# joybio/multiPrime

Measured on AMD Instinct MI355X. Metric: candidate x sequence coverage evals/s, higher is better.
Workload: dtype u32; 1 GPU; synthetic MSA 1048576 x 1000, k=18, v=1, 8 candidates/window, 950 windows, strict -c 2,3,-1 per GPU x 1 GPU(s) = BASELINE configs[3] itself (SURVEY 8d input 4; synthetic 1M x 1 kb; shape 1x1: row shards x window groups); rows_per_gpu=1048576, rows_total=1048576, cols=1000, k=18, variation=1, candidates_per_window=8, windows=950, parallelism=one GPU holds every row

## Files before the change

multiprime_amd/csrc/chainbody.hpp:

```cpp
#pragma once

#include "common.hpp"
#include "bitslice.hpp"

namespace mp {

struct EvalChainArgs {
    const unsigned long long *cols;
    const unsigned long long *excl;
    int nw, p0, k, v;
    const ChainItem *items;
    const uint32_t *events;
    const int32_t *cand_out;
    uint32_t sF, sR;
    unsigned long long *out;
    BlockMap map;
    PatchArgs patch;
    const ChainItem *neg_items;
    int n_neg;
    unsigned long long *clear;
    uint32_t n_clear;
};

__device__ __forceinline__ void clear_counters(unsigned long long *__restrict__ p, uint32_t n, unsigned bid, unsigned n_blocks) {
    if (!p) return;
    for (uint32_t i = bid * kBlock + threadIdx.x; i < n; i += n_blocks * kBlock) p[i] = 0ull;
}

template <int LV, int GW, int D, int NB>
__device__ __forceinline__ void chain_first_pass(uint32_t rem, const uint32_t *Pw, size_t nw32, unsigned long long sy_lo,
                                                 unsigned long long sy_hi, uint32_t sF, uint32_t sR, uint32_t (&t1)[GW],
                                                 uint32_t (&t2)[GW], uint32_t (&t3)[GW], uint32_t (&t4)[GW], uint32_t (&sf)[GW],
                                                 uint32_t (&sr)[GW]) {
#pragma unroll 1
    while (rem) {
        int js[D]; bool has[D];
        uint32_t ld[D][NB][GW], sys[D];
#pragma unroll
        for (int u = 0; u < D; u++) {
            has[u] = rem != 0u;
            js[u] = has[u] ? __builtin_ctz(rem) : js[0];
            rem &= rem - 1u;
            const int j = js[u];
            const uint32_t sy = (uint32_t)((j < 16 ? sy_lo : sy_hi) >> (4 * (j & 15))) & 15u;
            sys[u] = sy;
            const uint32_t *P = Pw + (size_t)j * 4 * nw32;
            if (NB == 4) {
#pragma unroll
                for (int b = 0; b < 4; b++)
#pragma unroll
                    for (int i = 0; i < GW; i++) ld[u][b][i] = P[b * nw32 + i];
            } else {
                const uint32_t second = sy & (sy - 1u);
                const size_t b0 = (size_t)__builtin_ctz(sy | 16u), b1 = (size_t)__builtin_ctz(second | 16u);
#pragma unroll
                for (int i = 0; i < GW; i++) {
                    ld[u][0][i] = P[b0 * nw32 + i];
                    if (NB == 2) ld[u][1][i] = P[b1 * nw32 + i];
                }
            }
        }
#pragma unroll
        for (int u = 0; u < D; u++) {
            if (!has[u]) break;
            const int j = js[u];
            uint32_t m[GW];
            if (NB == 4) {
                const uint32_t sy = sys[u];
                const uint32_t kA = (sy & 1u) ? 0xFFFFFFFFu : 0u, kC = (sy & 2u) ? 0xFFFFFFFFu : 0u;
                const uint32_t kG = (sy & 4u) ? 0xFFFFFFFFu : 0u, kT = (sy & 8u) ? 0xFFFFFFFFu : 0u;
#pragma unroll
                for (int i = 0; i < GW; i++) {
                    m[i] = ld[u][0][i] & kA;
                    m[i] = __builtin_amdgcn_bitop3_b32(ld[u][1][i], kC, m[i], kLutAndOr);
                    m[i] = __builtin_amdgcn_bitop3_b32(ld[u][2][i], kG, m[i], kLutAndOr);
                    m[i] = __builtin_amdgcn_bitop3_b32(ld[u][3][i], kT, m[i], kLutAndOr);
                }
            } else {
#pragma unroll
                for (int i = 0; i < GW; i++) m[i] = NB == 2 ? (ld[u][0][i] | ld[u][1][i]) : ld[u][0][i];
            }
#pragma unroll
            for (int i = 0; i < GW; i++) count_unmatched<LV>(t1[i], t2[i], t3[i], t4[i], m[i]);
            if (((sF | sR) >> j) & 1u) {
                const uint32_t fF = ((sF >> j) & 1u) ? 0xFFFFFFFFu : 0u, fR = ((sR >> j) & 1u) ? 0xFFFFFFFFu : 0u;
#pragma unroll
                for (int i = 0; i < GW; i++) {
                    sf[i] = __builtin_amdgcn_bitop3_b32(sf[i], m[i], fF, kLutOrNotAnd);
                    sr[i] = __builtin_amdgcn_bitop3_b32(sr[i], m[i], fR, kLutOrNotAnd);
                }
            }
        }
    }
}

template <int LV, int GW, int D>
__device__ __forceinline__ void eval_chain_block(const EvalChainArgs &A, uint32_t (&s_part)[kBlock / 64][12], const unsigned bid) {
    static_assert(GW <= 8, "plane rows are padded to multiples of 8 words");
    constexpr int CC = 8;
    const int patch_blocks = A.patch.n_blocks + A.patch.neg_blocks;
    const bool on_patch = (int)bid < patch_blocks;
    const bool negative = on_patch && (int)bid >= A.patch.n_blocks;
    int slice, item, word0;
    if (on_patch) {
        const int pb = (int)bid - (negative ? A.patch.n_blocks : 0);
        const int unit = __builtin_amdgcn_readfirstlane(pb * (kBlock / 64) + (int)(threadIdx.x >> 6));
        item = unit / A.patch.per_item;
        slice = unit % A.patch.per_item;
        if (item >= (negative ? A.n_neg : A.map.n_items)) return;
        word0 = (slice * 64 + (int)(threadIdx.x & 63)) * GW;
    } else {
        if (!map_block(A.map, bid - (unsigned)patch_blocks, slice, item)) return;
        word0 = (slice * kBlock + threadIdx.x) * GW;
    }
    const ChainItem it = negative ? A.neg_items[item] : A.items[item];
    const WordTile T = !on_patch ? column_tile(A.cols, A.excl, A.nw, A.p0, it.win, word0)
                                 : (negative ? plain_tile(A.patch, it.win, word0) : patch_tile(A.patch, it.win, word0));
    if (on_patch && slice * 64 * GW >= (int)T.stride) return;
    const size_t nw32 = T.stride;
    const bool live = T.live;
    static_assert(32 * GW < 1024, "three counts per register need 10 bits each");
    uint32_t acc[CC];
#pragma unroll
    for (int c = 0; c < CC; c++) acc[c] = 0;
    if (live) {
        uint32_t t1[GW], t2[GW], t3[GW], t4[GW], sf[GW], sr[GW];
#pragma unroll
        for (int i = 0; i < GW; i++) t1[i] = t2[i] = t3[i] = t4[i] = sf[i] = sr[i] = 0;
        const uint32_t *Pw = T.planes;
        const unsigned long long sy_lo = it.sym[0] | ((unsigned long long)it.sym[1] << 32);
        const unsigned long long sy_hi = it.sym[2] | ((unsigned long long)it.sym[3] << 32);
        chain_first_pass<LV, GW, D, 1>(it.pos1, Pw, nw32, sy_lo, sy_hi, A.sF, A.sR, t1, t2, t3, t4, sf, sr);
        chain_first_pass<LV, GW, (D + 1) / 2, 2>(it.pos2, Pw, nw32, sy_lo, sy_hi, A.sF, A.sR, t1, t2, t3, t4, sf, sr);
        chain_first_pass<LV, GW, (D + 3) / 4, 4>(it.pos4, Pw, nw32, sy_lo, sy_hi, A.sF, A.sR, t1, t2, t3, t4, sf, sr);
        uint32_t valid[GW];
        {
#pragma unroll
            for (int i = 0; i < GW; i++) valid[i] = T.mask[i] ^ T.mask_flip;
        }
        const uint32_t *ev = A.events + it.ev0;
        int e = 0;
        uint32_t evw = it.n_ev ? ev[0] : (1u << 8);
        uint32_t cur[GW];
        {
            const uint32_t *P = Pw + ((size_t)(evw & 255u) * 4 + (size_t)__builtin_ctz(((evw >> 8) & 15u) | 16u)) * nw32;
#pragma unroll
            for (int i = 0; i < GW; i++) cur[i] = P[i];
        }
#pragma unroll
        for (int s = 0; s < CC; s++) {
            if (s >= it.n_steps) break;
            if (s > 0) {
#pragma unroll 1
                while (e < it.n_ev && (int)(evw >> 16) == s) {
                    e++;
                    const uint32_t evn = e < it.n_ev ? ev[e] : evw;
                    uint32_t nxt[GW];
                    {
                        const uint32_t *P = Pw + ((size_t)(evn & 255u) * 4 + (size_t)__builtin_ctz(((evn >> 8) & 15u) | 16u)) * nw32;
#pragma unroll
                        for (int i = 0; i < GW; i++) nxt[i] = P[i];
                    }
                    const uint32_t j = evw & 255u;
#pragma unroll
                    for (int i = 0; i < GW; i++) count_plane<LV>(t1[i], t2[i], t3[i], t4[i], cur[i]);
                    if (((A.sF | A.sR) >> j) & 1u) {
                        const uint32_t fF = ((A.sF >> j) & 1u) ? 0xFFFFFFFFu : 0u, fR = ((A.sR >> j) & 1u) ? 0xFFFFFFFFu : 0u;
#pragma unroll
                        for (int i = 0; i < GW; i++) {
                            sf[i] = __builtin_amdgcn_bitop3_b32(sf[i], cur[i], fF, kLutOrAnd);
                            sr[i] = __builtin_amdgcn_bitop3_b32(sr[i], cur[i], fR, kLutOrAnd);
                        }
                    }
#pragma unroll
                    for (int i = 0; i < GW; i++) cur[i] = nxt[i];
                    evw = evn;
                }
            }
            uint32_t nP = 0, nF = 0, nR = 0;
#pragma unroll
            for (int i = 0; i < GW; i++) {
                const uint32_t far = LV == 1 ? t1[i] : (LV == 2 ? t2[i] : (LV == 3 ? t3[i] : t4[i]));
                nP += __popc(valid[i] & ~t1[i]);
                nF += __popc(__builtin_amdgcn_bitop3_b32(valid[i], far, sf[i], kLutAndNotNot));
                nR += __popc(__builtin_amdgcn_bitop3_b32(valid[i], far, sr[i], kLutAndNotNot));
            }
            acc[s] = nP | (nF << 10) | (nR << 20);
        }
    }
    uint32_t accP[CC], accF[CC], accR[CC];
#pragma unroll
    for (int c = 0; c < CC; c++) { accP[c] = acc[c] & 1023u; accF[c] = (acc[c] >> 10) & 1023u; accR[c] = acc[c] >> 20; }
    if (on_patch) wave_commit<GW>(accP, accF, accR, s_part[threadIdx.x >> 6], A.cand_out + it.cand0, A.out, negative);
    else block_commit<GW>(accP, accF, accR, s_part, A.cand_out + it.cand0, A.out);
}

constexpr int kPatchEvents = 16;
template <int LV>
__device__ __forceinline__ void eval_patch_wave(const EvalChainArgs &A, uint32_t *row, uint32_t *stash, const unsigned unit, const bool negative) {
    constexpr int CC = 8, GW = 1;
    const int lane = (int)(threadIdx.x & 63);
    const int item = __builtin_amdgcn_readfirstlane((int)(unit / (unsigned)A.patch.per_item)), slice = __builtin_amdgcn_readfirstlane((int)(unit % (unsigned)A.patch.per_item));
    if (item >= (negative ? A.n_neg : A.map.n_items)) return;
    const int word0 = slice * 64 + lane;
    const ChainItem it = negative ? A.neg_items[item] : A.items[item];
    const WordTile T = negative ? plain_tile(A.patch, it.win, word0) : patch_tile(A.patch, it.win, word0);
    if (slice * 64 >= (int)T.stride) return;
    const size_t nw32 = T.stride;
    const uint32_t *Pw = T.planes;
    const uint32_t *ev = A.events + it.ev0;
    const int n_ev = __builtin_amdgcn_readfirstlane((int)it.n_ev), n_steps = __builtin_amdgcn_readfirstlane((int)it.n_steps);
    const uint32_t evv = lane < n_ev ? ev[lane] : 0u;
    uint32_t acc[CC];
#pragma unroll
    for (int c = 0; c < CC; c++) acc[c] = 0;
    const uint32_t *Pl = T.live ? Pw : Pw - (word0 - slice * 64) ;
    uint32_t t1[GW] = {0}, t2[GW] = {0}, t3[GW] = {0}, t4[GW] = {0}, sf[GW] = {0}, sr[GW] = {0};
    const unsigned long long sy_lo = it.sym[0] | ((unsigned long long)it.sym[1] << 32);
    const unsigned long long sy_hi = it.sym[2] | ((unsigned long long)it.sym[3] << 32);
    chain_first_pass<LV, GW, 16, 1>(it.pos1, Pl, nw32, sy_lo, sy_hi, A.sF, A.sR, t1, t2, t3, t4, sf, sr);
    chain_first_pass<LV, GW, 8, 2>(it.pos2, Pl, nw32, sy_lo, sy_hi, A.sF, A.sR, t1, t2, t3, t4, sf, sr);
    chain_first_pass<LV, GW, 4, 4>(it.pos4, Pl, nw32, sy_lo, sy_hi, A.sF, A.sR, t1, t2, t3, t4, sf, sr);
    const uint32_t valid = T.live ? (T.mask[0] ^ T.mask_flip) : 0u;
    auto plane_of = [&](uint32_t evw) { return Pl + ((size_t)(evw & 255u) * 4 + (size_t)__builtin_ctz(((evw >> 8) & 15u) | 16u)) * nw32; };
    {
        uint32_t pl[kPatchEvents];
#pragma unroll
        for (int u = 0; u < kPatchEvents; u++) {
            const int e = n_ev ? (u < n_ev ? u : n_ev - 1) : 0;
            const uint32_t evw = n_ev ? (uint32_t)__builtin_amdgcn_readlane((int)evv, e) : (1u << 8);
            pl[u] = plane_of(evw)[0];
        }
#pragma unroll
        for (int u = 0; u < kPatchEvents; u++) stash[u * 64 + lane] = pl[u];
    }
    int e = 0;
#pragma unroll
    for (int s = 0; s < CC; s++) {
        if (s >= n_steps) break;
        if (s > 0) {
#pragma unroll 1
            while (e < n_ev) {
                const uint32_t evw = e < 64 ? (uint32_t)__builtin_amdgcn_readlane((int)evv, e) : ev[e];
                if ((int)(evw >> 16) != s) break;
                const uint32_t cur = e < kPatchEvents ? stash[e * 64 + lane] : plane_of(evw)[0];
                const uint32_t j = evw & 255u;
                count_plane<LV>(t1[0], t2[0], t3[0], t4[0], cur);
                if (((A.sF | A.sR) >> j) & 1u) {
                    const uint32_t fF = ((A.sF >> j) & 1u) ? 0xFFFFFFFFu : 0u, fR = ((A.sR >> j) & 1u) ? 0xFFFFFFFFu : 0u;
                    sf[0] = __builtin_amdgcn_bitop3_b32(sf[0], cur, fF, kLutOrAnd);
                    sr[0] = __builtin_amdgcn_bitop3_b32(sr[0], cur, fR, kLutOrAnd);
                }
                e++;
            }
        }
        const uint32_t far = LV == 1 ? t1[0] : (LV == 2 ? t2[0] : (LV == 3 ? t3[0] : t4[0]));
        const uint32_t nP = (uint32_t)__popc(valid & ~t1[0]);
        const uint32_t nF = (uint32_t)__popc(__builtin_amdgcn_bitop3_b32(valid, far, sf[0], kLutAndNotNot));
        const uint32_t nR = (uint32_t)__popc(__builtin_amdgcn_bitop3_b32(valid, far, sr[0], kLutAndNotNot));
        acc[s] = nP | (nF << 10) | (nR << 20);
    }
    uint32_t accP[CC], accF[CC], accR[CC];
#pragma unroll
    for (int c = 0; c < CC; c++) { accP[c] = acc[c] & 1023u; accF[c] = (acc[c] >> 10) & 1023u; accR[c] = acc[c] >> 20; }
    wave_commit<GW>(accP, accF, accR, row, A.cand_out + it.cand0, A.out, negative);
}

}
```

multiprime_amd/csrc/common.hpp:

```cpp
#pragma once

#include "../../include/mprime.h"

#include <hip/hip_runtime.h>

#include <algorithm>
#include <cstdarg>
#include <cstdio>
#include <cstdlib>
#include <cstring>
#include <numeric>
#include <utility>
#include <chrono>
#include <mutex>
#include <unordered_map>
#include <vector>

namespace mp {

constexpr int kBlock = 256;
constexpr uint32_t kEmpty = 0xFFFFFFFFu;
constexpr int kHashSlots = 4096;
constexpr int kHashLimit = 3584;
constexpr int kEvalCC = 8;
// ... 115 lines not shown
    uint32_t *pplanes = nullptr, *pvalid = nullptr;
    uint32_t *qplanes = nullptr, *qvalid = nullptr;
    bool qp_dirty = true;
    mp::PatchWin *pwin = nullptr;
    size_t pp_words = 0, pv_words = 0;
    int max_npw = 0;
    bool pp_dirty = true;
    unsigned long long *g_key = nullptr;
    uint32_t *g_cnt = nullptr, *g_min = nullptr;
    uint32_t *g_gap = nullptr;
    int32_t *g_idx = nullptr;
    int g_slots = 0;
    long long u_cap = 0, u_n = 0;
    uint32_t *u_b0 = nullptr, *u_b1 = nullptr, *u_g = nullptr;
    int32_t *u_count = nullptr, *u_first = nullptr, *labels = nullptr, *u_over = nullptr, *u_wcount = nullptr;
    int64_t *u_wbase = nullptr;
    unsigned long long *u_total = nullptr;
    std::vector<int64_t> h_wbase;
    std::vector<int32_t> h_wcount;
    double gate_threshold = 0;
    std::vector<uint8_t> h_wskip;
    uint8_t *dm_loss = nullptr;
    double *dm_dg = nullptr;
    std::vector<uint8_t> dm_loss_host;
    std::vector<double> dm_dg_host;
    unsigned long long *mask_f = nullptr, *mask_r = nullptr;
    size_t mask_words = 0;
    int n_masks = 0;
    int n_cand = 0, n_items = 0, n_padded = 0;
    mp::EvalItem *items = nullptr;
    uint4 *cand_n = nullptr;
    uint32_t *cand_symT = nullptr, *cand_diff = nullptr, *chain_events = nullptr;
    mp::ChainItem *chain_items = nullptr;
    void *x_items = nullptr;
    uint32_t *x_events = nullptr;
    int32_t *x_cand_out = nullptr;
    int x_n = 0, x_n_events = 0;
    int32_t *table_ids = nullptr;
    int n_chain = 0, n_table = 0, n_events = 0, max_steps = 0;
    std::vector<mp::ChainItem> h_chains;
    std::vector<uint32_t> h_events;
    std::vector<int32_t> h_cand_out;
    uint32_t *chain_prog = nullptr;
    size_t chain_prog_n = 0;
    mp::EvalForm form;
    mp::SlideBand *slide_bands = nullptr;
    uint32_t *slide_iters = nullptr, *slide_recs = nullptr;
    size_t slide_n_iters = 0;
    int slide_items = 0, slide_n_bands = 0, slide_max_items = 0, slide_ns = 0, slide_gw = 0;
    uint32_t slide_spos = 0, slide_fmask = 0, slide_rmask = 0, slide_fpos = 0, slide_rpos = 0;
    bool slide_fast = false;
    mp::ChainItem *chain_rest = nullptr;
    mp::ChainItem *chain_slid = nullptr;
    int n_rest = 0, rest_max_steps = 0;
    unsigned launch_seq = 0;
    int32_t *cand_out = nullptr;
    uint64_t sF = 0, sR = 0;
    unsigned long long *tmp_out = nullptr;
    int tmp_out_n = 0;
    struct PoolBlock { void *p; size_t bytes; hipEvent_t released; };
    std::vector<hipEvent_t> pool_events;
    std::unordered_map<void *, size_t> pool_live;
    std::vector<PoolBlock> pool;
    size_t pool_bytes = 0;
    long long pool_hits = 0, pool_misses = 0;
    int pool_on = -1;
    std::mutex pool_mu;
    unsigned long long *stats_buf = nullptr;
    size_t stats_buf_n = 0;
    std::vector<std::pair<hipEvent_t, hipEvent_t>> ev_busy, ev_free;
    double ev_ms = 0;
    std::vector<float> ev_samples, ev_last;
    int ev_n = 0;
    uint8_t *h_stage = nullptr;
    size_t h_stage_bytes = 0;
    bool h_stage_pinned = false;
    uint8_t *h_stats = nullptr;
    size_t h_stats_bytes = 0, stats_pending_f = 0, stats_pending_t = 0;
    bool h_stats_pinned = false;
    hipEvent_t stats_ev = nullptr;
    uint8_t *h_ring = nullptr;
    bool h_ring_pinned = false;
    hipEvent_t h_ring_ev[3] = {nullptr, nullptr, nullptr};
    uint8_t *sq_bytes = nullptr;
    int64_t *sq_roff = nullptr;
    unsigned long long *sq_code = nullptr, *sq_flag = nullptr;
    int64_t *sq_woff = nullptr;
    int32_t sq_n = 0;
    size_t sq_total = 0, sq_words = 0;
    std::vector<int64_t> sq_roff_host;
    int32_t *ot_out = nullptr;
    int64_t ot_n = 0;
    std::vector<uint8_t> ot_key;
    double ot_ms[4] = {0, 0, 0, 0};
    int64_t ot_counts[7] = {0, 0, 0, 0, 0, 0, 0};
    uint8_t *an_code = nullptr;
    uint32_t *an_kmer = nullptr;
    int32_t *an_table = nullptr;
    int32_t *an_col = nullptr, *an_colinv = nullptr;
    int32_t an_n = 0, an_L = 0, an_slots = 0;
    int32_t an_par[6] = {0, 0, 0, 0, 0, 0};
    double an_ms[5] = {0, 0, 0, 0, 0};
    int64_t an_counts[3] = {0, 0, 0};
    int32_t an_both = 0;
    uint8_t *cl_code = nullptr;
    int64_t *cl_off = nullptr;
// ... 127 lines not shown
```

multiprime_amd/csrc/evalslide.hip:

```cpp
#include "common.hpp"
#include "bitslice.hpp"
#include "slidecore.hpp"
#include "evalslide.hpp"
#include "chainbody.hpp"

using namespace mp;

namespace {

typedef unsigned int u32x4 __attribute__((ext_vector_type(4)));
typedef unsigned int u32x2 __attribute__((ext_vector_type(2)));

struct SlideKernArgs {
    SlideArgs A;
    const uint32_t *cols32;
    const uint32_t *excl32;
    int nw32;
    unsigned long long *out;
    int wc, wc_pad;
    int max_items;
    int n_slide_blocks;
    EvalChainArgs chain;
    unsigned long long *clear;
    uint32_t n_clear;
    int patch_words;
    unsigned long long *stamps;
};

template <int GW>
struct DevEnv {
    const SlideKernArgs &K;
    __amdgpu_buffer_rsrc_t rs_cols, rs_excl;
    int voff, lane;
    uint32_t row_bytes;
    bool live;
    uint32_t *ring;
    uint32_t *tab;
    uint32_t itv;
    uint32_t live_mask;

    __device__ __forceinline__ DevEnv(const SlideKernArgs &k) : K(k) {}
    __device__ __forceinline__ void progress(int quarter) const {
#ifndef SLIDE_NO_PRIO
        if (quarter <= 0) __builtin_amdgcn_s_setprio(3);
        else if (quarter == 1) __builtin_amdgcn_s_setprio(2);
        else if (quarter == 2) __builtin_amdgcn_s_setprio(1);
        else __builtin_amdgcn_s_setprio(0);
#endif
    }
    __device__ __forceinline__ void stamp(int i) const {
        if (K.stamps && threadIdx.x == 0) K.stamps[(size_t)blockIdx.x * 8 + i] = wall_clock64();
    }
    __device__ __forceinline__ SlideBand uband(int b) const {
        const SlideBand *p = K.A.bands + b;
        SlideBand r;
        r.w0 = __builtin_amdgcn_readfirstlane(p->w0); r.n_win = __builtin_amdgcn_readfirstlane(p->n_win);
        r.item0 = __builtin_amdgcn_readfirstlane(p->item0); r.n_items = __builtin_amdgcn_readfirstlane(p->n_items);
        r.iter0 = __builtin_amdgcn_readfirstlane(p->iter0); r.pad = 0;
        return r;
    }
    __device__ __forceinline__ void load_iters(int idx) { itv = K.A.iters[(size_t)idx + (size_t)lane]; }
    __device__ __forceinline__ uint32_t iter_word(int j) const { return (uint32_t)__builtin_amdgcn_readlane((int)itv, j); }
    typedef const uint32_t __attribute__((address_space(4))) * ConstWords;
    struct Rec { uint32_t w[8], sm_lo, sm_hi, flags; ConstWords p; };
    __device__ __forceinline__ Rec load_rec(int item) const {
        Rec r;
        r.p = (ConstWords)(K.A.recs + (size_t)__builtin_amdgcn_readfirstlane(item) * kSlideRec);
#pragma unroll
        for (int q = 0; q < 8; q++) r.w[q] = r.p[q];
        r.sm_lo = r.p[24]; r.sm_hi = r.p[25]; r.flags = r.p[28];
        return r;
    }
    __device__ __forceinline__ uint32_t rec_word(const Rec &r, int q) const {
        return q < 8 ? r.w[q] : (q == 24 ? r.sm_lo : (q == 25 ? r.sm_hi : (q == 28 ? r.flags : r.p[q])));
    }
    __device__ __forceinline__ uint32_t rec_word_dyn(const Rec &r, int q) const { return r.p[q]; }
    template <int AUX = 0>
    __device__ __forceinline__ void load(__amdgpu_buffer_rsrc_t rs, int soff, uint32_t (&d)[GW]) const {
        if constexpr (GW == 4) {
            const u32x4 v = __builtin_amdgcn_raw_buffer_load_b128(rs, voff, soff, AUX);
// ... 51 lines not shown
        asm volatile(
            "s_nop 1\n\t"
            "v_add_u32_dpp %0, %0, %0 row_ror:4 row_mask:0xf bank_mask:0x5\n\t"
            "v_add_u32_dpp %2, %2, %2 row_ror:4 row_mask:0xf bank_mask:0x5\n\t"
            "v_add_u32_dpp %4, %4, %4 row_ror:4 row_mask:0xf bank_mask:0x5\n\t"
            "v_add_u32_dpp %6, %6, %6 row_ror:4 row_mask:0xf bank_mask:0x5\n\t"
            "v_add_u32_dpp %8, %8, %8 row_ror:4 row_mask:0xf bank_mask:0x5\n\t"
            "v_add_u32_dpp %10, %10, %10 row_ror:4 row_mask:0xf bank_mask:0x5\n\t"
            "v_add_u32_dpp %0, %1, %1 row_ror:4 row_mask:0xf bank_mask:0xa\n\t"
            "v_add_u32_dpp %2, %3, %3 row_ror:4 row_mask:0xf bank_mask:0xa\n\t"
            "v_add_u32_dpp %4, %5, %5 row_ror:4 row_mask:0xf bank_mask:0xa\n\t"
            "v_add_u32_dpp %6, %7, %7 row_ror:4 row_mask:0xf bank_mask:0xa\n\t"
            "v_add_u32_dpp %8, %9, %9 row_ror:4 row_mask:0xf bank_mask:0xa\n\t"
            "v_add_u32_dpp %10, %11, %11 row_ror:4 row_mask:0xf bank_mask:0xa\n\t"
            "v_add_u32_dpp %0, %0, %0 row_ror:8 row_mask:0xf bank_mask:0x3\n\t"
            "v_add_u32_dpp %4, %4, %4 row_ror:8 row_mask:0xf bank_mask:0x3\n\t"
            "v_add_u32_dpp %8, %8, %8 row_ror:8 row_mask:0xf bank_mask:0x3\n\t"
            "v_add_u32_dpp %0, %2, %2 row_ror:8 row_mask:0xf bank_mask:0xc\n\t"
            "v_add_u32_dpp %4, %6, %6 row_ror:8 row_mask:0xf bank_mask:0xc\n\t"
            "v_add_u32_dpp %8, %10, %10 row_ror:8 row_mask:0xf bank_mask:0xc\n\t"
            "v_add_u32_dpp %0, %0, %0 quad_perm:[1,0,3,2] row_mask:0xf bank_mask:0xf\n\t"
            "v_add_u32_dpp %4, %4, %4 quad_perm:[1,0,3,2] row_mask:0xf bank_mask:0xf\n\t"
            "v_add_u32_dpp %8, %8, %8 quad_perm:[1,0,3,2] row_mask:0xf bank_mask:0xf\n\t"
            "v_add_u32_dpp %0, %0, %0 quad_perm:[2,3,0,1] row_mask:0xf bank_mask:0xf\n\t"
            "v_add_u32_dpp %4, %4, %4 quad_perm:[2,3,0,1] row_mask:0xf bank_mask:0xf\n\t"
            "v_add_u32_dpp %8, %8, %8 quad_perm:[2,3,0,1] row_mask:0xf bank_mask:0xf\n\t"
            "s_nop 1"
            : "+v"(x0), "+v"(x1), "+v"(x2), "+v"(x3), "+v"(x4), "+v"(x5), "+v"(x6), "+v"(x7), "+v"(x8), "+v"(x9), "+v"(x10), "+v"(x11));
        typedef unsigned int u32pair __attribute__((ext_vector_type(2)));
        const u32pair s01 = __builtin_amdgcn_permlane16_swap(x0, x4, false, false);
        const uint32_t a = s01.x + s01.y;
        const u32pair s22 = __builtin_amdgcn_permlane16_swap(x8, x8, false, false);
        const uint32_t b = s22.x + s22.y;
        const u32pair h = __builtin_amdgcn_permlane32_swap(a, b, false, false);
        const uint32_t tot = h.x + h.y;
        if (lane < 48 && (lane & 3) == 0) atomicAdd(&tab[idx * 12 + (lane >> 4) * 4 + ((lane >> 2) & 3)], tot);
    }
};

#ifndef SLIDE_MIN_WAVES
#define SLIDE_MIN_WAVES 1
#endif
template <int LV, int GW, bool FAST>
__global__ __launch_bounds__(kBlock, GW == 4 ? 1 : SLIDE_MIN_WAVES) void eval_slide_kernel(const SlideKernArgs K) {
    extern __shared__ __align__(16) uint32_t lds[];
    clear_counters(K.clear, K.n_clear, blockIdx.x, gridDim.x);
    if (K.stamps && threadIdx.x == 0) K.stamps[(size_t)blockIdx.x * 8] = wall_clock64();
    if ((int)blockIdx.x >= K.n_slide_blocks) {
        const unsigned pb = blockIdx.x - (unsigned)K.n_slide_blocks, wv = threadIdx.x >> 6;
#ifndef SLIDE_PATCH_PRIO
#define SLIDE_PATCH_PRIO 3
#endif
        __builtin_amdgcn_s_setprio(SLIDE_PATCH_PRIO);
        if (K.patch_words == 1) {
            const bool negative = (int)pb >= K.chain.patch.n_blocks;
            const unsigned unit = (pb - (negative ? (unsigned)K.chain.patch.n_blocks : 0u)) * (kBlock / 64) + wv;
            eval_patch_wave<LV>(K.chain, lds + wv * 12, lds + 64 + wv * (64 * kPatchEvents), unit, negative);
        } else {
            uint32_t(&s_part)[kBlock / 64][12] = *reinterpret_cast<uint32_t(*)[kBlock / 64][12]>(lds);
            eval_chain_block<LV, 8, 4>(K.chain, s_part, pb);
        }
        if (K.stamps && threadIdx.x == 0) K.stamps[(size_t)blockIdx.x * 8 + 7] = wall_clock64();
        return;
    }
    const int slice = (int)(blockIdx.x % (unsigned)K.wc_pad), band = (int)(blockIdx.x / (unsigned)K.wc_pad);
    if (slice >= K.wc) return;
    const int wv = (int)(threadIdx.x >> 6), lane = (int)(threadIdx.x & 63);
    const int ring_words = K.A.k * 64 * GW;
    uint32_t *tab = lds + (kBlock / 64) * ring_words;
    DevEnv<GW> env(K);
    env.lane = lane;
    env.ring = lds + wv * ring_words + lane * GW;
    env.tab = tab;
    env.itv = 0u;
    const int word0 = (slice * kBlock + (int)threadIdx.x) * GW;
    env.live = word0 < K.nw32;
    env.voff = env.live ? word0 * 4 : 0x7FFFFF00;
    env.live_mask = env.live ? 0xFFFFFFFFu : 0u;
    env.row_bytes = (uint32_t)K.nw32 * 4u;
    env.rs_cols = __builtin_amdgcn_make_buffer_rsrc(const_cast<uint32_t *>(K.cols32), 0, 0x7FFFFF00, 0x00020000);
    env.rs_excl = __builtin_amdgcn_make_buffer_rsrc(const_cast<uint32_t *>(K.excl32), 0, 0x7FFFFF00, 0x00020000);
    const SlideBand bd = env.uband(band);
    for (int i = (int)threadIdx.x; i < bd.n_items * 12; i += kBlock) tab[i] = 0u;
    __syncthreads();
    env.stamp(1);
    const bool wave_live = (slice * kBlock + wv * 64) * GW < K.nw32;
    if (wave_live) slide_band<LV, GW, true, false, FAST>(env, K.A, band);
    env.stamp(4);
    __syncthreads();
    env.stamp(5);
    int live_waves = 0;
    for (int w = 0; w < kBlock / 64; w++) live_waves += (slice * kBlock + w * 64) * GW < K.nw32 ? 1 : 0;
    const uint32_t rows = (uint32_t)live_waves * 64u * 32u * GW;
    const int n_entries = bd.n_items * 24;
    for (int i0 = (int)threadIdx.x; i0 < n_entries; i0 += 4 * kBlock) {
        int oc[4];
        uint32_t map[4];
#pragma unroll
        for (int u = 0; u < 4; u++) {
            const int i = i0 + u * kBlock, ic = i < n_entries ? i : (int)threadIdx.x;
            const uint32_t *rec = K.A.recs + (size_t)(bd.item0 + ic / 24) * kSlideRec;
            oc[u] = (int)rec[8 + (ic % 24) / 3];
            map[u] = rec[26];
        }
#pragma unroll
        for (int u = 0; u < 4; u++) {
            const int i = i0 + u * kBlock;
            if (i >= n_entries || oc[u] < 0) continue;
            const int item = i / 24, r = i % 24, t = r / 3, kind = r % 3;
            const int slot = (int)((map[u] >> (4 * t)) & 15u);
            const uint32_t *row = tab + item * 12;
            const uint32_t out1 = row[slot] & 0xFFFFu, outF = row[slot] >> 16, outR = (row[8 + (slot >> 1)] >> (16 * (slot & 1))) & 0xFFFFu;
            const uint32_t val = kind == 0 ? rows - out1 : out1 - (kind == 1 ? outF : outR);
            if (val) atomicAdd(&K.out[(size_t)oc[u] * 3 + kind], (unsigned long long)val);
        }
    }
    env.stamp(6);
}

typedef void (*SlideFn)(const SlideKernArgs);

}

namespace mp {

void free_slide(mp_ctx *c) {
    dev_free(c, &c->slide_bands, (size_t)c->slide_n_bands);
    dev_free(c, &c->slide_iters, c->slide_n_iters);
    dev_free(c, &c->slide_recs, (size_t)c->slide_items * kSlideRec);
    dev_free(c, &c->chain_rest, (size_t)c->n_rest);
    dev_free(c, &c->chain_slid, (size_t)c->slide_items);
    c->slide_items = c->slide_n_bands = c->slide_max_items = 0;
    c->slide_n_iters = 0;
    c->n_rest = c->rest_max_steps = 0;
}

int upload_eval_slide(mp_ctx *c, const std::vector<ChainItem> &chains, const std::vector<uint32_t> &events, const std::vector<int32_t> &cand_out) {
    free_slide(c);
    const char *se = getenv("MP_EVAL_SLIDE");
    if (chains.empty() || c->v > 3 || c->k <= c->v || (se ? atoi(se) != 1 : c->n_pad <= 262144)) return MP_OK;
    const int nw32 = c->n_pad / 32, n_cols = c->n_chunks * 32;
    if (((unsigned long long)n_cols * 4ull + 1ull) * (unsigned long long)nw32 * 4ull >= 0x7FFFFFFFull) return MP_OK;
    if ((unsigned long long)c->n_win * (unsigned long long)nw32 * 4ull >= 0x7FFFFFFFull) return MP_OK;
    int gw = 2;
    if (const char *e = getenv("MP_SLIDE_GW")) { const int g = atoi(e); if (g == 1 || g == 2 || g == 4) gw = g; }
    const int wc = (nw32 + kBlock * gw - 1) / (kBlock * gw), wc_pad = wc >= 8 ? (wc + 7) / 8 * 8 : wc;
    const int span = chains.back().win - chains.front().win + 1;
    std::vector<SlideChainIn> in(chains.size());
    for (size_t i = 0; i < chains.size(); i++) {
        const ChainItem &ch = chains[i];
        in[i] = SlideChainIn{ch.win, ch.cand0, ch.n_steps, ch.ev0, ch.n_ev, {ch.sym[0], ch.sym[1], ch.sym[2], ch.sym[3]}};
    }
    const size_t ring_bytes = (size_t)(kBlock / 64) * ((size_t)c->k * 64 * gw) * sizeof(uint32_t), lds_cu = 160 * 1024;
    int resident = (int)std::min<size_t>(4, std::max<size_t>(1, lds_cu / (ring_bytes + 1024)));
    if (gw == 4) resident = 1;
    SlidePlan P;
    for (;; resident--) {
        const int per_round = std::max(1, 256 * resident / std::max(1, wc_pad));
        int band = (span + per_round - 1) / per_round;
        for (int r = 2; band > 96; r++) band = (span + per_round * r - 1) / (per_round * r);
        band = std::max(8, band);
        if (const char *e = getenv("MP_SLIDE_BAND")) band = std::max(1, atoi(e));
        if (!build_slide_plan(in, events, cand_out, c->k, (uint32_t)c->sF, (uint32_t)c->sR, c->p0, n_cols, band, (uint32_t)nw32 * 4u, true, P)) return MP_OK;
        const size_t need = ring_bytes + (size_t)P.max_items_band * 12 * sizeof(uint32_t);
        if (resident <= 1 || need * (size_t)resident <= lds_cu) break;
    }
    P.iters.resize(P.iters.size() + 64, 0u);
    int rc;
    if ((rc = dev_alloc(c, &c->slide_bands, P.bands.size()))) return rc;
    c->slide_n_bands = (int)P.bands.size();
    if ((rc = dev_alloc(c, &c->slide_iters, P.iters.size()))) return rc;
    c->slide_n_iters = P.iters.size();
    c->slide_items = (int)P.item_of.size();
    if ((rc = dev_alloc(c, &c->slide_recs, P.recs.size()))) return rc;
    HIPCK(c, hipMemcpy(c->slide_bands, P.bands.data(), sizeof(SlideBand) * P.bands.size(), hipMemcpyHostToDevice));
    HIPCK(c, hipMemcpy(c->slide_iters, P.iters.data(), sizeof(uint32_t) * P.iters.size(), hipMemcpyHostToDevice));
    HIPCK(c, hipMemcpy(c->slide_recs, P.recs.data(), sizeof(uint32_t) * P.recs.size(), hipMemcpyHostToDevice));
    c->slide_max_items = P.max_items_band;
    c->slide_ns = P.ns; c->slide_spos = P.spos; c->slide_fmask = P.fmask; c->slide_rmask = P.rmask;
    c->slide_fast = slide_strict_lists(c->k, (uint32_t)c->sF, (uint32_t)c->sR, c->slide_fpos, c->slide_rpos);
    if (const char *e = getenv("MP_SLIDE_STRICT")) { if (atoi(e) == 0) c->slide_fast = false; }
    c->slide_gw = gw;
    {
        std::vector<ChainItem> slid;
        for (int32_t i : P.item_of) slid.push_back(chains[(size_t)i]);
        if ((rc = dev_alloc(c, &c->chain_slid, slid.size()))) return rc;
        HIPCK(c, hipMemcpy(c->chain_slid, slid.data(), sizeof(ChainItem) * slid.size(), hipMemcpyHostToDevice));
    }
    if (!P.rest.empty()) {
        std::vector<ChainItem> rest;
        for (int32_t i : P.rest) { rest.push_back(chains[(size_t)i]); c->rest_max_steps = std::max(c->rest_max_steps, (int)chains[(size_t)i].n_steps); }
        if ((rc = dev_alloc(c, &c->chain_rest, rest.size()))) return rc;
        c->n_rest = (int)rest.size();
        HIPCK(c, hipMemcpy(c->chain_rest, rest.data(), sizeof(ChainItem) * rest.size(), hipMemcpyHostToDevice));
    }
    return MP_OK;
}

int launch_eval_slide(mp_ctx *c, unsigned long long *device_out, const EvalChainArgs *patch, int patch_blocks, int patch_words,
                      unsigned long long *clear, uint32_t n_clear) {
#define SLIDE_ROW(LV, F) {eval_slide_kernel<LV, 1, F>, eval_slide_kernel<LV, 2, F>, eval_slide_kernel<LV, 4, F>}
    static const SlideFn fn[2][4][3] = {{SLIDE_ROW(1, false), SLIDE_ROW(2, false), SLIDE_ROW(3, false), SLIDE_ROW(4, false)},
                                        {SLIDE_ROW(1, true), SLIDE_ROW(2, true), SLIDE_ROW(3, true), SLIDE_ROW(4, true)}};
#undef SLIDE_ROW
    const int gw = c->slide_gw, gi = gw == 4 ? 2 : gw - 1;
    const int nw32 = c->n_pad / 32;
    SlideKernArgs K;
    K.A = SlideArgs{c->slide_bands, c->slide_iters, c->slide_recs, c->k, c->p0, c->slide_ns, c->slide_spos, c->slide_fmask, c->slide_rmask,
                    (uint32_t)nw32 * 4u, c->slide_fpos, c->slide_rpos, 0u, 0u};
    if (c->slide_fast) slide_strict_distinct(c->slide_fpos, c->slide_rpos, K.A.dpos, K.A.dshape);
    K.cols32 = reinterpret_cast<const uint32_t *>(c->cols);
    K.excl32 = reinterpret_cast<const uint32_t *>(c->excl);
    K.nw32 = nw32;
    K.out = device_out;
    K.wc = (nw32 + kBlock * gw - 1) / (kBlock * gw);
    K.wc_pad = K.wc >= 8 ? (K.wc + 7) / 8 * 8 : K.wc;
    K.max_items = c->slide_max_items;
    K.n_slide_blocks = c->slide_n_bands * K.wc_pad;
    if (patch) K.chain = *patch;
    else { memset(&K.chain, 0, sizeof K.chain); patch_blocks = 0; }
    K.chain.clear = nullptr; K.chain.n_clear = 0;
    K.clear = clear; K.n_clear = n_clear;
    K.patch_words = patch_words;
    K.stamps = nullptr;
    const char *stamp_file = getenv("MP_EXPERIMENT_STAMPS");
    const size_t n_stamp = ((size_t)K.n_slide_blocks + (size_t)patch_blocks) * 8;
    if (stamp_file) {
        HIPCK(c, hipMalloc(&K.stamps, n_stamp * sizeof(unsigned long long)));
        HIPCK(c, hipMemsetAsync(K.stamps, 0, n_stamp * sizeof(unsigned long long), c->stream));
    }
    size_t lds = ((size_t)(kBlock / 64) * ((size_t)c->k * 64 * gw) + (size_t)c->slide_max_items * 12) * sizeof(uint32_t);
    if (patch_blocks) lds = std::max(lds, (size_t)(64 + (kBlock / 64) * 64 * kPatchEvents) * sizeof(uint32_t));
    if (lds > 160 * 1024) return fail(c, MP_ERR_ARG, "sliding evaluation: a band needs %zu bytes of LDS", lds);
    SlideFn f = fn[c->slide_fast ? 1 : 0][c->v][gi];
    if (lds > 48 * 1024) HIPCK(c, hipFuncSetAttribute(reinterpret_cast<const void *>(f), hipFuncAttributeMaxDynamicSharedMemorySize, (int)lds));
    hipLaunchKernelGGL(f, dim3((unsigned)K.n_slide_blocks + (unsigned)patch_blocks), dim3(kBlock), lds, c->stream, K);
    HIPCK(c, hipGetLastError());
    if (stamp_file) {
        std::vector<unsigned long long> h(n_stamp + 2);
        HIPCK(c, hipStreamSynchronize(c->stream));
        HIPCK(c, hipMemcpy(h.data() + 2, K.stamps, n_stamp * sizeof(unsigned long long), hipMemcpyDeviceToHost));
        HIPCK(c, hipFree(K.stamps));
        h[0] = (unsigned long long)K.n_slide_blocks; h[1] = (unsigned long long)patch_blocks;
        if (FILE *fo = fopen(stamp_file, "wb")) { fwrite(h.data(), sizeof(unsigned long long), h.size(), fo); fclose(fo); }
    }
    return MP_OK;
}

}
```

Measured before the change: 66790 billion evals/s.

## Fuse positive and negative patch units into one signed evaluation pass

```diff
diff --git a/multiprime_amd/csrc/chainbody.hpp b/multiprime_amd/csrc/chainbody.hpp
--- a/multiprime_amd/csrc/chainbody.hpp
+++ b/multiprime_amd/csrc/chainbody.hpp
@@ -20,18 +20,24 @@
     int n_neg;
     unsigned long long *clear;
     uint32_t n_clear;
+    const uint32_t *slid_bits;
 };
+
+#ifndef PATCH_SIGNED
+#define PATCH_SIGNED 1
+#endif
 
 __device__ __forceinline__ void clear_counters(unsigned long long *__restrict__ p, uint32_t n, unsigned bid, unsigned n_blocks) {
     if (!p) return;
     for (uint32_t i = bid * kBlock + threadIdx.x; i < n; i += n_blocks * kBlock) p[i] = 0ull;
 }
 
-template <int LV, int GW, int D, int NB>
+template <int LV, int GW, int D, int NB, bool PAIR = false>
 __device__ __forceinline__ void chain_first_pass(uint32_t rem, const uint32_t *Pw, size_t nw32, unsigned long long sy_lo,
                                                  unsigned long long sy_hi, uint32_t sF, uint32_t sR, uint32_t (&t1)[GW],
                                                  uint32_t (&t2)[GW], uint32_t (&t3)[GW], uint32_t (&t4)[GW], uint32_t (&sf)[GW],
-                                                 uint32_t (&sr)[GW]) {
+                                                 uint32_t (&sr)[GW], const uint32_t *Pw2 = nullptr) {
+    static_assert(!PAIR || GW % 2 == 0, "a pair of tiles: half of the words of each");
 #pragma unroll 1
     while (rem) {
         int js[D]; bool has[D];
@@ -44,19 +50,20 @@
             const int j = js[u];
             const uint32_t sy = (uint32_t)((j < 16 ? sy_lo : sy_hi) >> (4 * (j & 15))) & 15u;
             sys[u] = sy;
-            const uint32_t *P = Pw + (size_t)j * 4 * nw32;
+            const uint32_t *P = Pw + (size_t)j * 4 * nw32, *P2 = PAIR ? Pw2 + (size_t)j * 4 * nw32 : nullptr;
+            auto word = [&](size_t b, int i) { return PAIR && i >= GW / 2 ? P2[b * nw32 + (i - GW / 2)] : P[b * nw32 + i]; };
             if (NB == 4) {
 #pragma unroll
                 for (int b = 0; b < 4; b++)
 #pragma unroll
-                    for (int i = 0; i < GW; i++) ld[u][b][i] = P[b * nw32 + i];
+                    for (int i = 0; i < GW; i++) ld[u][b][i] = word((size_t)b, i);
             } else {
                 const uint32_t second = sy & (sy - 1u);
                 const size_t b0 = (size_t)__builtin_ctz(sy | 16u), b1 = (size_t)__builtin_ctz(second | 16u);
 #pragma unroll
                 for (int i = 0; i < GW; i++) {
-                    ld[u][0][i] = P[b0 * nw32 + i];
-                    if (NB == 2) ld[u][1][i] = P[b1 * nw32 + i];
+                    ld[u][0][i] = word(b0, i);
+                    if (NB == 2) ld[u][1][i] = word(b1, i);
                 }
             }
         }
@@ -94,21 +101,59 @@
     }
 }
 
-template <int LV, int GW, int D>
-__device__ __forceinline__ void eval_chain_block(const EvalChainArgs &A, uint32_t (&s_part)[kBlock / 64][12], const unsigned bid) {
+constexpr int kPatchRowSigned = 24;
+template <int GW>
+__device__ __forceinline__ void wave_commit_signed(const uint32_t (&acc_pos)[8], const uint32_t (&acc_neg)[8], uint32_t *row, const int32_t *cand_out,
+                                                   unsigned long long *out) {
+    constexpr int CC = 8;
+    static_assert(64 * 32 * GW < 65536, "packed wave sums must fit 16 bits");
+    const int lane = threadIdx.x & 63;
+#pragma unroll
+    for (int side = 0; side < 2; side++) {
+        const uint32_t(&acc)[8] = side ? acc_neg : acc_pos;
+        uint32_t vals[3 * CC];
+#pragma unroll
+        for (int c = 0; c < CC; c++) { vals[3 * c] = acc[c] & 1023u; vals[3 * c + 1] = (acc[c] >> 10) & 1023u; vals[3 * c + 2] = acc[c] >> 20; }
+#pragma unroll
+        for (int q = 0; q < 3 * CC / 2; q++) {
+            const uint32_t tot = wave_sum_lane63(vals[2 * q] | (vals[2 * q + 1] << 16));
+            if (lane == 63) row[side * 12 + q] = tot;
+        }
+    }
+    __builtin_amdgcn_fence(__ATOMIC_RELEASE, "wavefront");
+    __builtin_amdgcn_wave_barrier();
+    __builtin_amdgcn_fence(__ATOMIC_ACQUIRE, "wavefront");
+    if (lane < 3 * CC) {
+        const int c = lane / 3, r = lane % 3;
+        auto field = [&](const uint32_t *w, int idx) { return (w[idx >> 1] >> (16 * (idx & 1))) & 0xFFFFu; };
+        const uint32_t pos = r ? field(row, lane) - field(row, 3 * c) : field(row, lane);
+        const uint32_t neg = r ? field(row + 12, lane) - field(row + 12, 3 * c) : field(row + 12, lane);
+        const int oc = cand_out[c];
+        if (oc >= 0 && pos != neg) atomicAdd(&out[(size_t)oc * 3 + r], (unsigned long long)pos - (unsigned long long)neg);
+    }
+}
+
+template <int LV, int GW, int D, bool PAIR = false>
+__device__ __forceinline__ void eval_chain_block(const EvalChainArgs &A, uint32_t (&s_part)[kBlock / 64][12], const unsigned bid, uint32_t *pair_row = nullptr) {
     static_assert(GW <= 8, "plane rows are padded to multiples of 8 words");
-    constexpr int CC = 8;
+    constexpr int CC = 8, H = PAIR ? GW / 2 : GW;
     const int patch_blocks = A.patch.n_blocks + A.patch.neg_blocks;
-    const bool on_patch = (int)bid < patch_blocks;
-    const bool negative = on_patch && (int)bid >= A.patch.n_blocks;
+    const bool on_patch = PAIR || (int)bid < patch_blocks;
+    const bool negative = !PAIR && on_patch && (int)bid >= A.patch.n_blocks;
     int slice, item, word0;
     if (on_patch) {
         const int pb = (int)bid - (negative ? A.patch.n_blocks : 0);
         const int unit = __builtin_amdgcn_readfirstlane(pb * (kBlock / 64) + (int)(threadIdx.x >> 6));
-        item = unit / A.patch.per_item;
-        slice = unit % A.patch.per_item;
-        if (item >= (negative ? A.n_neg : A.map.n_items)) return;
-        word0 = (slice * 64 + (int)(threadIdx.x & 63)) * GW;
+        if (PAIR) {
+            item = unit % A.map.n_items;
+            slice = unit / A.map.n_items;
+            if (slice >= A.patch.per_item) return;
+        } else {
+            item = unit / A.patch.per_item;
+            slice = unit % A.patch.per_item;
+            if (item >= (negative ? A.n_neg : A.map.n_items)) return;
+        }
+        word0 = (slice * 64 + (int)(threadIdx.x & 63)) * H;
     } else {
         if (!map_block(A.map, bid - (unsigned)patch_blocks, slice, item)) return;
         word0 = (slice * kBlock + threadIdx.x) * GW;
@@ -116,37 +161,51 @@
     const ChainItem it = negative ? A.neg_items[item] : A.items[item];
     const WordTile T = !on_patch ? column_tile(A.cols, A.excl, A.nw, A.p0, it.win, word0)
                                  : (negative ? plain_tile(A.patch, it.win, word0) : patch_tile(A.patch, it.win, word0));
-    if (on_patch && slice * 64 * GW >= (int)T.stride) return;
+    if (on_patch && slice * 64 * H >= (int)T.stride) return;
     const size_t nw32 = T.stride;
     const bool live = T.live;
+    const uint32_t *Pq = nullptr, *Mq = nullptr;
+    bool slides = false;
+    if (PAIR) {
+        slides = __builtin_amdgcn_readfirstlane((int)((A.slid_bits[item >> 5] >> (item & 31)) & 1u)) != 0;
+        const WordTile Q = plain_tile(A.patch, it.win, word0);
+        Pq = slides ? Q.planes : T.planes;
+        Mq = Q.mask;
+    }
     static_assert(32 * GW < 1024, "three counts per register need 10 bits each");
-    uint32_t acc[CC];
+    constexpr int NH = PAIR ? 2 : 1;
+    uint32_t acc[CC], acc_neg[PAIR ? CC : 1];
 #pragma unroll
     for (int c = 0; c < CC; c++) acc[c] = 0;
+    if constexpr (PAIR) {
+#pragma unroll
+        for (int c = 0; c < CC; c++) acc_neg[c] = 0;
+    }
     if (live) {
         uint32_t t1[GW], t2[GW], t3[GW], t4[GW], sf[GW], sr[GW];
 #pragma unroll
         for (int i = 0; i < GW; i++) t1[i] = t2[i] = t3[i] = t4[i] = sf[i] = sr[i] = 0;
         const uint32_t *Pw = T.planes;
+        auto plane_words = [&](uint32_t evw, uint32_t (&d)[GW]) {
+            const size_t off = ((size_t)(evw & 255u) * 4 + (size_t)__builtin_ctz(((evw >> 8) & 15u) | 16u)) * nw32;
+#pragma unroll
+            for (int i = 0; i < GW; i++) d[i] = PAIR && i >= H ? Pq[off + (i - H)] : Pw[off + i];
+        };
         const unsigned long long sy_lo = it.sym[0] | ((unsigned long long)it.sym[1] << 32);
         const unsigned long long sy_hi = it.sym[2] | ((unsigned long long)it.sym[3] << 32);
-        chain_first_pass<LV, GW, D, 1>(it.pos1, Pw, nw32, sy_lo, sy_hi, A.sF, A.sR, t1, t2, t3, t4, sf, sr);
-        chain_first_pass<LV, GW, (D + 1) / 2, 2>(it.pos2, Pw, nw32, sy_lo, sy_hi, A.sF, A.sR, t1, t2, t3, t4, sf, sr);
-        chain_first_pass<LV, GW, (D + 3) / 4, 4>(it.pos4, Pw, nw32, sy_lo, sy_hi, A.sF, A.sR, t1, t2, t3, t4, sf, sr);
+        chain_first_pass<LV, GW, D, 1, PAIR>(it.pos1, Pw, nw32, sy_lo, sy_hi, A.sF, A.sR, t1, t2, t3, t4, sf, sr, Pq);
+        chain_first_pass<LV, GW, (D + 1) / 2, 2, PAIR>(it.pos2, Pw, nw32, sy_lo, sy_hi, A.sF, A.sR, t1, t2, t3, t4, sf, sr, Pq);
+        chain_first_pass<LV, GW, (D + 3) / 4, 4, PAIR>(it.pos4, Pw, nw32, sy_lo, sy_hi, A.sF, A.sR, t1, t2, t3, t4, sf, sr, Pq);
         uint32_t valid[GW];
         {
 #pragma unroll
-            for (int i = 0; i < GW; i++) valid[i] = T.mask[i] ^ T.mask_flip;
+            for (int i = 0; i < GW; i++) valid[i] = PAIR && i >= H ? (slides ? Mq[i - H] : 0u) : T.mask[i] ^ T.mask_flip;
         }
         const uint32_t *ev = A.events + it.ev0;
         int e = 0;
         uint32_t evw = it.n_ev ? ev[0] : (1u << 8);
         uint32_t cur[GW];
-        {
-            const uint32_t *P = Pw + ((size_t)(evw & 255u) * 4 + (size_t)__builtin_ctz(((evw >> 8) & 15u) | 16u)) * nw32;
-#pragma unroll
-            for (int i = 0; i < GW; i++) cur[i] = P[i];
-        }
+        plane_words(evw, cur);
 #pragma unroll
         for (int s = 0; s < CC; s++) {
             if (s >= it.n_steps) break;
@@ -156,11 +215,7 @@
                     e++;
                     const uint32_t evn = e < it.n_ev ? ev[e] : evw;
                     uint32_t nxt[GW];
-                    {
-                        const uint32_t *P = Pw + ((size_t)(evn & 255u) * 4 + (size_t)__builtin_ctz(((evn >> 8) & 15u) | 16u)) * nw32;
-#pragma unroll
-                        for (int i = 0; i < GW; i++) nxt[i] = P[i];
-                    }
+                    plane_words(evn, nxt);
                     const uint32_t j = evw & 255u;
 #pragma unroll
                     for (int i = 0; i < GW; i++) count_plane<LV>(t1[i], t2[i], t3[i], t4[i], cur[i]);
@@ -177,16 +232,22 @@
                     evw = evn;
                 }
             }
-            uint32_t nP = 0, nF = 0, nR = 0;
+            uint32_t nP[NH] = {}, nF[NH] = {}, nR[NH] = {};
 #pragma unroll
             for (int i = 0; i < GW; i++) {
                 const uint32_t far = LV == 1 ? t1[i] : (LV == 2 ? t2[i] : (LV == 3 ? t3[i] : t4[i]));
-                nP += __popc(valid[i] & ~t1[i]);
-                nF += __popc(__builtin_amdgcn_bitop3_b32(valid[i], far, sf[i], kLutAndNotNot));
-                nR += __popc(__builtin_amdgcn_bitop3_b32(valid[i], far, sr[i], kLutAndNotNot));
-            }
-            acc[s] = nP | (nF << 10) | (nR << 20);
-        }
+                const int h = PAIR && i >= H ? 1 : 0;
+                nP[h] += __popc(valid[i] & ~t1[i]);
+                nF[h] += __popc(__builtin_amdgcn_bitop3_b32(valid[i], far, sf[i], kLutAndNotNot));
+                nR[h] += __popc(__builtin_amdgcn_bitop3_b32(valid[i], far, sr[i], kLutAndNotNot));
+            }
+            acc[s] = nP[0] | (nF[0] << 10) | (nR[0] << 20);
+            if constexpr (PAIR) acc_neg[s] = nP[1] | (nF[1] << 10) | (nR[1] << 20);
+        }
+    }
+    if constexpr (PAIR) {
+        wave_commit_signed<H>(acc, acc_neg, pair_row, A.cand_out + it.cand0, A.out);
+        return;
     }
     uint32_t accP[CC], accF[CC], accR[CC];
 #pragma unroll
@@ -266,4 +327,85 @@
     wave_commit<GW>(accP, accF, accR, row, A.cand_out + it.cand0, A.out, negative);
 }
 
-}
+template <int LV>
+__device__ __forceinline__ void eval_patch_wave_signed(const EvalChainArgs &A, uint32_t *row, uint32_t *stash, const unsigned unit) {
+    constexpr int CC = 8, GW = 1;
+    const int lane = (int)(threadIdx.x & 63);
+    const int item = __builtin_amdgcn_readfirstlane((int)(unit / (unsigned)A.patch.per_item)), slice = __builtin_amdgcn_readfirstlane((int)(unit % (unsigned)A.patch.per_item));
+    if (item >= A.map.n_items) return;
+    const int word0 = slice * 64 + lane;
+    const bool slides = __builtin_amdgcn_readfirstlane((int)((A.slid_bits[item >> 5] >> (item & 31)) & 1u)) != 0;
+    const ChainItem it = A.items[item];
+    const WordTile T = patch_tile(A.patch, it.win, word0), Q = plain_tile(A.patch, it.win, word0);
+    if (slice * 64 >= (int)T.stride) return;
+    const size_t nw32 = T.stride;
+    const uint32_t *ev = A.events + it.ev0;
+    const int n_ev = __builtin_amdgcn_readfirstlane((int)it.n_ev), n_steps = __builtin_amdgcn_readfirstlane((int)it.n_steps);
+    const uint32_t evv = lane < n_ev ? ev[lane] : 0u;
+    const int back = T.live ? 0 : word0 - slice * 64;
+    const uint32_t *Pl[2] = {T.planes - back, slides ? Q.planes - back : T.planes - back};
+    const uint32_t valid[2] = {T.live ? (T.mask[0] ^ T.mask_flip) : 0u, slides && Q.live ? (Q.mask[0] ^ Q.mask_flip) : 0u};
+    uint32_t t1[2] = {0, 0}, t2[2] = {0, 0}, t3[2] = {0, 0}, t4[2] = {0, 0}, sf[2] = {0, 0}, sr[2] = {0, 0};
+    const unsigned long long sy_lo = it.sym[0] | ((unsigned long long)it.sym[1] << 32);
+    const unsigned long long sy_hi = it.sym[2] | ((unsigned long long)it.sym[3] << 32);
+    chain_first_pass<LV, 2, 16, 1, true>(it.pos1, Pl[0], nw32, sy_lo, sy_hi, A.sF, A.sR, t1, t2, t3, t4, sf, sr, Pl[1]);
+    chain_first_pass<LV, 2, 8, 2, true>(it.pos2, Pl[0], nw32, sy_lo, sy_hi, A.sF, A.sR, t1, t2, t3, t4, sf, sr, Pl[1]);
+    chain_first_pass<LV, 2, 4, 4, true>(it.pos4, Pl[0], nw32, sy_lo, sy_hi, A.sF, A.sR, t1, t2, t3, t4, sf, sr, Pl[1]);
+    auto plane_off = [&](uint32_t evw) { return ((size_t)(evw & 255u) * 4 + (size_t)__builtin_ctz(((evw >> 8) & 15u) | 16u)) * nw32; };
+    {
+        uint32_t pl[2][kPatchEvents];
+#pragma unroll
+        for (int u = 0; u < kPatchEvents; u++) {
+            const int e = n_ev ? (u < n_ev ? u : n_ev - 1) : 0;
+            const uint32_t evw = n_ev ? (uint32_t)__builtin_amdgcn_readlane((int)evv, e) : (1u << 8);
+            const size_t o = plane_off(evw);
+            pl[0][u] = Pl[0][o];
+            pl[1][u] = Pl[1][o];
+        }
+#pragma unroll
+        for (int t = 0; t < 2; t++)
+#pragma unroll
+            for (int u = 0; u < kPatchEvents; u++) stash[(t * kPatchEvents + u) * 64 + lane] = pl[t][u];
+    }
+    uint32_t acc[2][CC];
+#pragma unroll
+    for (int c = 0; c < CC; c++) acc[0][c] = acc[1][c] = 0;
+    int e = 0;
+#pragma unroll
+    for (int s = 0; s < CC; s++) {
+        if (s >= n_steps) break;
+        if (s > 0) {
+#pragma unroll 1
+            while (e < n_ev) {
+                const uint32_t evw = e < 64 ? (uint32_t)__builtin_amdgcn_readlane((int)evv, e) : ev[e];
+                if ((int)(evw >> 16) != s) break;
+                uint32_t cur[2];
+                if (e < kPatchEvents) { cur[0] = stash[e * 64 + lane]; cur[1] = stash[(kPatchEvents + e) * 64 + lane]; }
+                else { const size_t o = plane_off(evw); cur[0] = Pl[0][o]; cur[1] = Pl[1][o]; }
+                const uint32_t j = evw & 255u;
+#pragma unroll
+                for (int t = 0; t < 2; t++) count_plane<LV>(t1[t], t2[t], t3[t], t4[t], cur[t]);
+                if (((A.sF | A.sR) >> j) & 1u) {
+                    const uint32_t fF = ((A.sF >> j) & 1u) ? 0xFFFFFFFFu : 0u, fR = ((A.sR >> j) & 1u) ? 0xFFFFFFFFu : 0u;
+#pragma unroll
+                    for (int t = 0; t < 2; t++) {
+                        sf[t] = __builtin_amdgcn_bitop3_b32(sf[t], cur[t], fF, kLutOrAnd);
+                        sr[t] = __builtin_amdgcn_bitop3_b32(sr[t], cur[t], fR, kLutOrAnd);
+                    }
+                }
+                e++;
+            }
+        }
+#pragma unroll
+        for (int t = 0; t < 2; t++) {
+            const uint32_t far = LV == 1 ? t1[t] : (LV == 2 ? t2[t] : (LV == 3 ? t3[t] : t4[t]));
+            const uint32_t nP = (uint32_t)__popc(valid[t] & ~t1[t]);
+            const uint32_t nF = (uint32_t)__popc(__builtin_amdgcn_bitop3_b32(valid[t], far, sf[t], kLutAndNotNot));
+            const uint32_t nR = (uint32_t)__popc(__builtin_amdgcn_bitop3_b32(valid[t], far, sr[t], kLutAndNotNot));
+            acc[t][s] = nP | (nF << 10) | (nR << 20);
+        }
+    }
+    wave_commit_signed<GW>(acc[0], acc[1], row, A.cand_out + it.cand0, A.out);
+}
+
+}
diff --git a/multiprime_amd/csrc/common.hpp b/multiprime_amd/csrc/common.hpp
--- a/multiprime_amd/csrc/common.hpp
+++ b/multiprime_amd/csrc/common.hpp
@@ -191,6 +191,8 @@
     bool slide_fast = false;
     mp::ChainItem *chain_rest = nullptr;
     mp::ChainItem *chain_slid = nullptr;
+    uint32_t *chain_slid_bits = nullptr;
+    size_t n_slid_words = 0;
     int n_rest = 0, rest_max_steps = 0;
     unsigned launch_seq = 0;
     int32_t *cand_out = nullptr;
diff --git a/multiprime_amd/csrc/evalslide.hip b/multiprime_amd/csrc/evalslide.hip
--- a/multiprime_amd/csrc/evalslide.hip
+++ b/multiprime_amd/csrc/evalslide.hip
@@ -26,6 +26,10 @@
     int patch_words;
     unsigned long long *stamps;
 };
+
+constexpr int kPatchHeadSigned = 128;
+constexpr size_t kPatchLdsSigned = (size_t)(kPatchHeadSigned + (kBlock / 64) * 2 * 64 * kPatchEvents) * sizeof(uint32_t);
+static_assert((kBlock / 64) * kPatchRowSigned <= kPatchHeadSigned, "the waves' rows fit in front of the stashes");
 
 template <int GW>
 struct DevEnv {
@@ -183,13 +187,16 @@
 #define SLIDE_PATCH_PRIO 3
 #endif
         __builtin_amdgcn_s_setprio(SLIDE_PATCH_PRIO);
-        if (K.patch_words == 1) {
+        if (PATCH_SIGNED && K.patch_words == 1 && K.chain.slid_bits) {
+            eval_patch_wave_signed<LV>(K.chain, lds + wv * kPatchRowSigned, lds + kPatchHeadSigned + wv * (2 * 64 * kPatchEvents), pb * (kBlock / 64) + wv);
+        } else if (K.patch_words == 1) {
             const bool negative = (int)pb >= K.chain.patch.n_blocks;
             const unsigned unit = (pb - (negative ? (unsigned)K.chain.patch.n_blocks : 0u)) * (kBlock / 64) + wv;
             eval_patch_wave<LV>(K.chain, lds + wv * 12, lds + 64 + wv * (64 * kPatchEvents), unit, negative);
         } else {
             uint32_t(&s_part)[kBlock / 64][12] = *reinterpret_cast<uint32_t(*)[kBlock / 64][12]>(lds);
-            eval_chain_block<LV, 8, 4>(K.chain, s_part, pb);
+            if (PATCH_SIGNED && K.chain.slid_bits) eval_chain_block<LV, 8, 4, true>(K.chain, s_part, pb, lds + wv * kPatchRowSigned);
+            else eval_chain_block<LV, 8, 4>(K.chain, s_part, pb);
         }
         if (K.stamps && threadIdx.x == 0) K.stamps[(size_t)blockIdx.x * 8 + 7] = wall_clock64();
         return;
@@ -261,6 +268,8 @@
     dev_free(c, &c->slide_recs, (size_t)c->slide_items * kSlideRec);
     dev_free(c, &c->chain_rest, (size_t)c->n_rest);
     dev_free(c, &c->chain_slid, (size_t)c->slide_items);
+    dev_free(c, &c->chain_slid_bits, c->n_slid_words);
+    c->n_slid_words = 0;
     c->slide_items = c->slide_n_bands = c->slide_max_items = 0;
     c->slide_n_iters = 0;
     c->n_rest = c->rest_max_steps = 0;
@@ -317,6 +326,11 @@
         for (int32_t i : P.item_of) slid.push_back(chains[(size_t)i]);
         if ((rc = dev_alloc(c, &c->chain_slid, slid.size()))) return rc;
         HIPCK(c, hipMemcpy(c->chain_slid, slid.data(), sizeof(ChainItem) * slid.size(), hipMemcpyHostToDevice));
+        std::vector<uint32_t> bits((chains.size() + 31) / 32, 0u);
+        for (int32_t i : P.item_of) bits[(size_t)i >> 5] |= 1u << (i & 31);
+        if ((rc = dev_alloc(c, &c->chain_slid_bits, bits.size()))) return rc;
+        c->n_slid_words = bits.size();
+        HIPCK(c, hipMemcpy(c->chain_slid_bits, bits.data(), sizeof(uint32_t) * bits.size(), hipMemcpyHostToDevice));
     }
     if (!P.rest.empty()) {
         std::vector<ChainItem> rest;
@@ -351,6 +365,22 @@
     if (patch) K.chain = *patch;
     else { memset(&K.chain, 0, sizeof K.chain); patch_blocks = 0; }
     K.chain.clear = nullptr; K.chain.n_clear = 0;
+    K.chain.slid_bits = nullptr;
+    bool signed_units = false;
+#if PATCH_SIGNED
+    const PatchArgs half = patch_blocks && patch_words != 1 ? patch_args(c, 4, K.chain.map.n_items, 64) : PatchArgs{};
+    if (patch_blocks && c->chain_slid_bits && (patch_words == 1 || half.n_blocks <= patch_blocks)) {
+        signed_units = true;
+        K.chain.slid_bits = c->chain_slid_bits;
+        if (patch_words == 1) {
+            patch_blocks -= K.chain.patch.neg_blocks;
+        } else {
+            K.chain.patch.per_item = half.per_item;
+            K.chain.patch.n_blocks = patch_blocks = half.n_blocks;
+        }
+        K.chain.patch.neg_blocks = 0;
+    }
+#endif
     K.clear = clear; K.n_clear = n_clear;
     K.patch_words = patch_words;
     K.stamps = nullptr;
@@ -361,7 +391,7 @@
         HIPCK(c, hipMemsetAsync(K.stamps, 0, n_stamp * sizeof(unsigned long long), c->stream));
     }
     size_t lds = ((size_t)(kBlock / 64) * ((size_t)c->k * 64 * gw) + (size_t)c->slide_max_items * 12) * sizeof(uint32_t);
-    if (patch_blocks) lds = std::max(lds, (size_t)(64 + (kBlock / 64) * 64 * kPatchEvents) * sizeof(uint32_t));
+    if (patch_blocks) lds = std::max(lds, signed_units && patch_words == 1 ? kPatchLdsSigned :(size_t)(64 + (kBlock / 64) * 64 * kPatchEvents) * sizeof(uint32_t));
     if (lds > 160 * 1024) return fail(c, MP_ERR_ARG, "sliding evaluation: a band needs %zu bytes of LDS", lds);
     SlideFn f = fn[c->slide_fast ? 1 : 0][c->v][gi];
     if (lds > 48 * 1024) HIPCK(c, hipFuncSetAttribute(reinterpret_cast<const void *>(f), hipFuncAttributeMaxDynamicSharedMemorySize, (int)lds));
```

Result: no change. 66600 billion evals/s (-0.3%).
